# MIT-SPARK/Kimera-Semantics

Measured on NVIDIA H100. Metric: depth_frames_per_s, higher is better.
Workload: dtype f32

## Files before the change

### kimera_semantics_b200/csrc/ksg_api.cu

```cuda
#include <cuda_runtime.h>
#include <cub/cub.cuh>

#include <algorithm>
#include <climits>
#include <cmath>
#include <cstdio>
#include <cstdlib>
#include <cstring>
#include <memory>
#include <numeric>
#include <string>
#include <type_traits>
#include <unordered_map>
#include <unordered_set>
#include <utility>
#include <vector>

#include "../../include/ksg.h"
#include "ksg_kernels.cuh"
#include "ksg_chain.cuh"
#include "ksg_hot.cuh"
#include "ksg_bundle_order.cuh"
#include "ksg_fast.cuh"
#include "ksg_fast3.cuh"
// ... 136 lines not shown

}

struct ksg_integrator {
  ksg_config cfg{};
  DevCfg dc{};
  int device = 0;
  int sm_count = 132;
  cudaStream_t own_stream = nullptr;
  std::string err;
  int deferred_status = 0;

  MapRef map{};
  uint32_t ht_cap = 0;
  Luts h_luts{};
  Luts* d_luts = nullptr;
  Counters* d_cnt = nullptr;
  Counters* h_cnt = nullptr;
  int frame_stamp = 0;
  int64_t num_blocks = 0;
  int64_t last_blocks_touched = 0;

  int cap_points = 0;
  float4 *pt_pC = nullptr, *pt_pG = nullptr;
  uint8_t *pt_label = nullptr, *pt_flags = nullptr;
  uint32_t* pt_color = nullptr;
  uint64_t* pt_key = nullptr;
  uint8_t* flags8 = nullptr;
  int* pix_list = nullptr;
  int* point_of_seq = nullptr;
  uint32_t *sq_keys = nullptr, *sq_keys_out = nullptr;
  uint32_t *iota = nullptr;

  int *start_next = nullptr, *start_min = nullptr, *start_max = nullptr;
  uint32_t *start_table = nullptr;
  int *s_base = nullptr, *s_visits = nullptr;
  uint32_t *s_hmin = nullptr, *s_hmax = nullptr;
  uint8_t *clear_ff = nullptr, *clear_00 = nullptr;
  uint64_t set_offset = 0;
  int64_t reset_counter = 0;
  int* cast_seq = nullptr;
  float4* ray_param = nullptr;
  uint8_t *ray_label = nullptr, *ray_flags = nullptr;
  uint32_t* ray_color = nullptr;
  int* nsteps = nullptr;
  RayState* ray_state = nullptr;
  long long* ext_off = nullptr;
  Obs3 o3{};

  uint64_t* ks_sorted = nullptr;
  uint32_t* seq_sorted = nullptr;
  int *bstart = nullptr, *bundle_f = nullptr;
  float *hist = nullptr, *tmp = nullptr, *tmp4 = nullptr;
  uint64_t* b_key = nullptr;
  long long* b_base = nullptr;
  std::vector<std::pair<int, uint32_t>> bord_phases;
  uint32_t* bord_hash = nullptr;
  int* bundle_f2 = nullptr;
  int* bord_scratch = nullptr;
  unsigned long long* d_scan_tot = nullptr;
  BordBuf bord{};

  bool hot_enabled = false;
  HotSeg* d_hot_segs = nullptr;
  HotSeg* h_hot_segs = nullptr;
  int *d_hot_counts = nullptr;
  int *d_hot_chunk_seg = nullptr, *h_hot_chunk_seg = nullptr, *d_hot_guess = nullptr;
// ... 321 lines not shown
}
int finish_frame(ksg_integrator* h, ksg_frame_stats* stats) {
  while (h->n_pend > 1) { const int rc = finish_oldest(h, nullptr); if (rc) return rc; }
  if (h->n_pend == 1) return finish_oldest(h, stats);
  if (stats) fill_stats(h, stats);
  if (h->deferred_status) return h->fail(h->deferred_status, err_text(h->deferred_status));
  return KSG_OK;
}
int complete_frames(ksg_integrator* h) {
  KSG_CUDA(cudaSetDevice(h->device));
  KSG_CUDA(cudaDeviceSynchronize());
  return finish_frame(h, nullptr);
}

int advance_sets(ksg_integrator* h, cudaStream_t s) {
  if ((++h->reset_counter) >= h->cfg.clear_checks_every_n_frames) {
    h->reset_counter = 0;
    if (++h->set_offset >= 10000) {
      h->set_offset = 0;
      KSG_CUDA(cudaMemsetAsync(h->start_table, 0xFF, sizeof(uint32_t) * kSetSize, s));
      KSG_CUDA(cudaMemsetAsync(h->o3.table, 0xFF, sizeof(uint32_t) * kSetSize, s));
    }
  }
  return KSG_OK;
}

int integrate_fast(ksg_integrator* h, const InputDesc& in, const FrameIn& fin, const Xform& T, int cap, cudaStream_t s,
                   ksg_frame_stats* stats) {
  const bool sorted = h->cfg.integration_order_mode == KSG_ORDER_SORTED;
  { const int rcs = advance_sets(h, s); if (rcs) return rcs; }
  FastFrame f{};
  f.cfg = h->dc; f.T = T; f.in = fin; f.in.pix_list = nullptr; f.in.point_of_seq = nullptr;
  f.luts = h->d_luts; f.cnt = h->d_cnt; f.fc = h->d_fc; f.map = h->map;
  f.sb = StartBuf{h->start_next, h->start_min, h->start_max, h->start_table};
  f.set_offset = h->set_offset;
  f.capacity = cap;
  f.n_count_blocks = (cap + kCountBlock - 1) / kCountBlock;
  f.vec_ok = in.d_depth ? (((uintptr_t)in.d_depth % 16 == 0 && (uintptr_t)in.d_label_img % 4 == 0) ? 1 : 0) : 0;
  f.frame_stamp = h->frame_stamp;
  f.profile = (h->profiling && !h->profile_marks_only) ? 1 : 0;
  f.prof_marks = h->profiling ? 1 : 0;
  f.seq_of_i = sorted ? h->seq_of_i : nullptr;
  f.block_cnt = h->blk_cnt; f.block_off = h->blk_off; f.warp_cnt = h->warp_cnt; f.warp_off = h->warp_off;
  f.pt_pG = h->pt_pG; f.pt_label = h->pt_label; f.pt_flags = h->pt_flags; f.pt_color = h->pt_color; f.pt_key = h->pt_key;
  f.cast_flag = h->flags8;
  f.cast_seq = h->cast_seq; f.ray_param = h->ray_param; f.ray_label = h->ray_label; f.ray_flags = h->ray_flags; f.ray_color = h->ray_color;
  f.ray_state = h->ray_state; f.ext_off = h->ext_off;
  f.rec_cap = h->rec_cap; f.keys = h->keys32;
  f.tile_cnt = h->tile_cnt; f.tile_slot = h->tile_slot; f.tile_list = h->tile_list; f.tile_cap = h->tile_cap;
  f.o3 = h->o3;
  f.rayrec = h->rayrec; f.blk_run = h->blk_run;
  f.wl_listed = h->wl;
  f.wl_list[0] = h->wl + h->cap_points; f.wl_list[1] = h->wl + 2 * (size_t)h->cap_points;
  f.log_head = h->d_log_head; f.log_prior = h->d_log_prior; f.log_cap = h->log_cap;
  f.s_base = h->s_base; f.s_hmin = h->s_hmin; f.s_hmax = h->s_hmax; f.s_visits = h->s_visits;
  f.mixed_list = h->mixed_list; f.m_list = h->m_list;

  if (h->profiling) {
    cudaEventRecord(h->ev[0], s);
    KSG_CUDA(cudaMemsetAsync(h->d_fc->dbg, 0, sizeof(h->d_fc->dbg), s));
  }
  KSG_CUDA(cudaMemsetAsync(h->clear_ff, 0xFF, (size_t)kSetSize * 16, s));
  KSG_CUDA(cudaMemsetAsync(h->clear_00, 0x00, (size_t)kSetSize * 13, s));
  KSG_CUDA(cudaMemsetAsync(h->start_min, 0x7F, sizeof(int) * kSetSize, s));
  const int B = 256;
  ++h->n_launches;
  if (in.d_depth) k_fast_count<<<f.n_count_blocks, 256, 0, s>>>(f);
  else k_fast_reset<<<1, 1, 0, s>>>(f);
  if (sorted) {
    h->n_launches += 3;
    if (in.d_depth) k_fast_sqnorm<<<f.n_count_blocks, 256, 0, s>>>(f, h->sq_keys);
    else k_fast_sqnorm_points<<<grid_for(cap, B), B, 0, s>>>(f, h->sq_keys);
    k_fast_pad_keys<<<grid_for(cap, B), B, 0, s>>>(h->d_cnt, cap, h->sq_keys);
    size_t tb = h->cub_temp_bytes;
    ++h->n_libcalls;
    KSG_CUDA(cub::DeviceRadixSort::SortPairs(h->cub_temp, tb, h->sq_keys, h->sq_keys_out, h->iota, (uint32_t*)h->point_of_seq, cap, 0, 32, s));
    k_fast_invert_perm<<<grid_for(cap, B), B, 0, s>>>(h->d_cnt, (const uint32_t*)h->point_of_seq, h->seq_of_i);
  }
  ++h->n_launches;
  if (in.d_depth) k_fast_classify<true><<<f.n_count_blocks, 256, 0, s>>>(f);
  else k_fast_classify<false><<<grid_for(cap, B), B, 0, s>>>(f);
  ++h->n_launches;
  k_fast_start_eval3<<<(cap + kEvalBlock - 1) / kEvalBlock, kEvalBlock, 0, s>>>(f);
  if (h->profiling) cudaEventRecord(h->ev[1], s);
  {
    int max_sweeps = h->cap_points + 2;
    void* args[] = {(void*)&f, (void*)&max_sweeps};
    ++h->n_launches;
    KSG_CUDA(cudaLaunchCooperativeKernel((const void*)k_fast_solve3, dim3(h->solve_grid), dim3(h->solve_threads), args,
                                         (size_t)h->solve_smem, s));
  }
  if (h->profiling) cudaEventRecord(h->ev[2], s);
  {
    ApplySrc src{};
    src.param = h->ray_param; src.label = h->ray_label; src.color = h->ray_color; src.tmp = nullptr;
// ... 472 lines not shown
    h->h_luts.dynamic_label[l] = cfg->dynamic_label[l];
  }
  for (int i = 0; i < 1024; ++i) { h->h_luts.c2l_keys[i] = 0xFFFFFFFFu; h->h_luts.c2l_vals[i] = 0; }
  KSG_CUDA(res.device(&h->d_luts, 1));
  KSG_CUDA(cudaMemcpy(h->d_luts, &h->h_luts, sizeof(Luts), cudaMemcpyHostToDevice));

  h->ht_cap = 1024;
  while (h->ht_cap < 2u * (uint32_t)cfg->max_blocks) h->ht_cap <<= 1;
  if ((unsigned long long)h->ht_cap * dc.tiles_per_block >= (1ull << 32)) return h->fail(KSG_ERR_INVALID_ARGUMENT, "max_blocks too large");
  h->map.ht_mask = h->ht_cap - 1;
  h->map.max_blocks = cfg->max_blocks;
  h->map.new_cap = cfg->max_blocks;
  KSG_CUDA(res.device(&h->map.ht_keys, h->ht_cap));
  KSG_CUDA(res.device(&h->map.ht_slot, h->ht_cap));
  KSG_CUDA(res.device(&h->map.touched_stamp, h->ht_cap));
  KSG_CUDA(res.device(&h->map.touched_list, h->ht_cap));
  KSG_CUDA(res.device(&h->map.new_list, (size_t)cfg->max_blocks));
  KSG_CUDA(res.device(&h->map.slot_key, (size_t)cfg->max_blocks));
  KSG_CUDA(res.device(&h->map.pool, (size_t)dc.block_stride * (size_t)cfg->max_blocks));
  KSG_CUDA(res.device(&h->d_cnt, 1));
  KSG_CUDA(res.pinned(&h->h_cnt_base, 2));
  std::memset(h->h_cnt_base, 0, 2 * sizeof(Counters));
  h->h_cnt = h->h_cnt_base;
  for (int i = 0; i < 2; ++i) {
    KSG_CUDA(res.event(&h->ev_frame_s[i], cudaEventDisableTiming));
    KSG_CUDA(res.event(&h->ev_copy[i], cudaEventDisableTiming));
    KSG_CUDA(res.event(&h->ev_free[i], cudaEventDisableTiming));
  }
  KSG_CUDA(res.stream(&h->copy_stream));

  const size_t N = (size_t)cfg->max_points;
  h->cap_points = cfg->max_points;
  const bool fast = cfg->integrator_type == KSG_INTEGRATOR_FAST;
  KSG_CUDA(res.device(&h->pt_pC, N)); KSG_CUDA(res.device(&h->pt_pG, N));
  KSG_CUDA(res.device(&h->pt_label, N)); KSG_CUDA(res.device(&h->pt_flags, N));
  KSG_CUDA(res.device(&h->pt_color, N)); KSG_CUDA(res.device(&h->pt_key, N));
  KSG_CUDA(res.device(&h->flags8, 2 * N));
  KSG_CUDA(res.device(&h->pix_list, N));
  KSG_CUDA(res.device(&h->iota, N));
  k_iota<<<grid_for((long long)N, 256), 256>>>(h->iota, (int)N);
  if (cfg->integration_order_mode == KSG_ORDER_SORTED) {
    KSG_CUDA(res.device(&h->point_of_seq, N)); KSG_CUDA(res.device(&h->sq_keys, N)); KSG_CUDA(res.device(&h->sq_keys_out, N));
  }
  KSG_CUDA(res.device(&h->ray_param, N)); KSG_CUDA(res.device(&h->ray_flags, N)); KSG_CUDA(res.device(&h->nsteps, N));
  long long rec_cap = cfg->max_updates > 0 ? cfg->max_updates : (fast ? std::max<long long>(4ll << 20, 64ll * (long long)N) : (64ll << 20));
  if (fast) {
    KSG_CUDA(res.device(&h->start_next, N)); KSG_CUDA(res.device(&h->start_table, kSetSize));
    KSG_CUDA(res.device(&h->clear_ff, (size_t)kSetSize * 16));
    KSG_CUDA(res.device(&h->clear_00, (size_t)kSetSize * 13));
    h->s_base = (int*)h->clear_ff; h->start_max = h->s_base + kSetSize; h->s_hmin = (uint32_t*)(h->start_max + kSetSize);
    h->o3.head = (int*)(h->clear_ff + (size_t)kSetSize * 12);
    h->o3.slot_cnt = (int*)h->clear_00;
    h->s_hmax = (uint32_t*)(h->clear_00 + (size_t)kSetSize * 5); h->s_visits = (int*)(h->clear_00 + (size_t)kSetSize * 9);
    KSG_CUDA(res.device(&h->start_min, kSetSize));
    KSG_CUDA(res.device(&h->cast_seq, N));
    KSG_CUDA(res.device(&h->ray_label, N)); KSG_CUDA(res.device(&h->ray_color, N));
    KSG_CUDA(res.device(&h->ray_state, N)); KSG_CUDA(res.device(&h->ext_off, N * kExtSegs));
    long long ext = cfg->max_ray_steps > 0 ? cfg->max_ray_steps : std::max<long long>(16ll << 20, 64ll * (long long)N);
    Obs3& o3 = h->o3;
    o3.ext_base = (long long)N * kH0;
    o3.cand_cap = o3.ext_base + ext;
    if (o3.cand_cap >= 0x7FFFFFFFll) { o3.cand_cap = 0x7FFFFFFEll; }
    KSG_CUDA(res.device(&o3.cand, (size_t)o3.cand_cap));
    o3.ovf_cap = (int)std::min<long long>(std::max<long long>(1ll << 20, 4ll * (long long)N), 1ll << 28);
    KSG_CUDA(res.device(&o3.ovf, (size_t)o3.ovf_cap));
    KSG_CUDA(res.device(&o3.bkt, (size_t)kSetSize * kBkt3));
    KSG_CUDA(res.device(&o3.stamp_max, 2 * (size_t)kSetSize)); o3.stamp_min = o3.stamp_max + kSetSize;
    KSG_CUDA(res.device(&o3.table, kSetSize));
    KSG_CUDA(res.device(&h->rayrec, N));
    KSG_CUDA(res.device(&h->wl, 3 * N));
    KSG_CUDA(res.device(&h->mixed_list, N)); KSG_CUDA(res.device(&h->m_list, N));
    KSG_CUDA(res.device(&h->blk_run, (size_t)(o3.cand_cap / 16 + 16)));
  } else {
    KSG_CUDA(res.device(&h->ks_sorted, N)); KSG_CUDA(res.device(&h->seq_sorted, N));
    KSG_CUDA(res.device(&h->bstart, 2 * N)); KSG_CUDA(res.device(&h->bundle_f, N));
    KSG_CUDA(res.device(&h->hist, N * dc.C)); KSG_CUDA(res.device(&h->tmp, (N + 1) * dc.C));
    KSG_CUDA(res.device(&h->b_key, N)); KSG_CUDA(res.device(&h->b_base, N));
    KSG_CUDA(res.device(&h->d_scan_tot, 16));
    h->voxel_apply = cfg->apply_mode == 0 && !knobs.tile_apply;
    if (h->voxel_apply) {
      h->vq.long_cap = 4 * (rec_cap / kLongLen) + 64;
      h->vq.long_len = kLongLen;
      if (dc.C <= 32) {
        KSG_CUDA(res.device(&h->tmp4, (N + 1) * (size_t)((dc.C + 3) & ~3)));
// ... 1505 lines not shown
```

### kimera_semantics_b200/csrc/ksg_fast.cuh

```cuda
#pragma once
#include "ksg_kernels.cuh"

namespace ksg {

static constexpr int kCountBlock = 1024;
static constexpr int kEvalBlock = 512;
static constexpr int kSolveThreads = 1024;
static constexpr int kFastKeyCap = 4096;
static constexpr int kGroupThreads = 512;
static constexpr int kFastApplyThreads = 256;
static constexpr int kRecVoxMax = 1 << kRecVoxBits;
static constexpr int kTimelineSlots = 64;

struct FastCounters {
  unsigned int ticket_count, ticket_eval;
  unsigned int gridbar;
  int sweep_base;
  int sweeps_last;
  int tile_cursor;
  int n_tile_list;
  int pool_base;
  unsigned long long rec_cursor;
  int ovf_count;
  int n_mixed;
  int m_cursor;
  int log_count;
  int item_cursor;
  int wl_claim[4];
  int wl_count[4];
  long long timeline[kTimelineSlots];
  long long dbg[16];
};

struct TileDesc { uint32_t tk; int n; long long off; };
struct __align__(16) FastTile { long long off; int slot, tile, bx, by, bz, pad; };
struct __align__(16) FastItem { int tile, vox, lo, len; };

struct VoxelUpdate { int bx, by, bz; uint32_t lin_label; float dist, wgt; uint32_t rgba, srgba; };

struct StartBuf {
  int* next;
  int* smin;
  int* smax;
  const uint32_t* table;
};

struct Cand;
struct OvfEnt;
struct RayRec;
struct Obs3 {
  Cand* cand;
  long long ext_base, cand_cap;
  int* slot_cnt;
  uint64_t* bkt;
  int* head;
  OvfEnt* ovf;
  int ovf_cap;
  uint64_t* stamp_max;
  uint64_t* stamp_min;
  uint32_t* table;
};

struct FastFrame {
  DevCfg cfg;
  Xform T;
  FrameIn in;
  const Luts* luts;
  Counters* cnt;
  FastCounters* fc;
  MapRef map;
  StartBuf sb;
  uint64_t set_offset;
  int capacity;
  int n_count_blocks;
  int vec_ok;
  int frame_stamp;
  int profile;
  int prof_marks;
  const int* seq_of_i;
  int* block_cnt; int* block_off;
  int* warp_cnt; int* warp_off;
  float4* pt_pG; uint8_t* pt_label; uint8_t* pt_flags; uint32_t* pt_color; uint64_t* pt_key; uint8_t* cast_flag;
  int* cast_seq; float4* ray_param; uint8_t* ray_label; uint8_t* ray_flags; uint32_t* ray_color;
  RayState* ray_state; long long* ext_off;
  long long rec_cap;
  uint32_t* keys;
  int* tile_cnt;
  int* tile_slot;
  TileDesc* tile_list; long long tile_cap;
  Obs3 o3;
  RayRec* rayrec;
  int* blk_run;
  int* wl_listed;
  int* wl_list[2];
  VoxelUpdate* log_head; float* log_prior; int log_cap;
  int* s_visits;
  uint32_t *s_hmin, *s_hmax;
  int* s_base;
  int* mixed_list;
  int* m_list;
};

__device__ __forceinline__ int inv_mixed_index(int i, int n) {
  const int groups = n / 1024;
  if (groups * 1024 <= i) return i;
  return (i % 1024) * groups + i / 1024;
}

__device__ __forceinline__ int block_scan_array(const int* a, int* out, int n) {
  __shared__ int s_w[32];
  __shared__ int s_total;
  const int tid = threadIdx.x, lane = tid & 31, wid = tid >> 5;
  const int nthreads = blockDim.x, nwarps = nthreads >> 5;
  const int per = (((n + nthreads - 1) / nthreads) + 3) & ~3;
  const int i0 = min(n, tid * per), i1 = min(n, i0 + per);
// ... 32 lines not shown

__device__ __forceinline__ void load_depth4(const float* __restrict__ depth, int p0, int P, int vec_ok, float d[4], int& npx) {
  npx = P - p0; if (npx > 4) npx = 4; if (npx < 0) npx = 0;
  if (npx == 4 && vec_ok) { const float4 v = __ldg((const float4*)(depth + p0)); d[0] = v.x; d[1] = v.y; d[2] = v.z; d[3] = v.w; }
  else { for (int k = 0; k < 4; ++k) d[k] = (k < npx) ? __ldg(depth + p0 + k) : 0.0f; }
}

__global__ void __launch_bounds__(256) k_fast_count(FastFrame f) {
  __shared__ int s_w[8];
  __shared__ int s_last;
  const int tid = threadIdx.x, lane = tid & 31, wid = tid >> 5;
  const int p0 = blockIdx.x * kCountBlock + tid * 4;
  float d[4]; int npx;
  load_depth4(f.in.depth, p0, f.capacity, f.vec_ok, d, npx);
  int c = 0;
  for (int k = 0; k < 4; ++k) c += (k < npx && isfinite(d[k])) ? 1 : 0;
  for (int o = 16; o > 0; o >>= 1) c += __shfl_down_sync(0xffffffffu, c, o);
  if (lane == 0) s_w[wid] = c;
  __syncthreads();
  if (tid == 0) {
    int t = 0; for (int w = 0; w < 8; ++w) t += s_w[w];
    __stcg(&f.block_cnt[blockIdx.x], t);
    __threadfence();
    s_last = (atomicAdd(&f.fc->ticket_count, 1u) == (unsigned)(f.n_count_blocks - 1));
  }
  __syncthreads();
  if (!s_last) return;
  __threadfence();
  const int total = block_scan_array(f.block_cnt, f.block_off, f.n_count_blocks);
  if (tid == 0) { frame_counters_reset(f.cnt, total); f.fc->ticket_count = 0; }
}
__global__ void k_fast_reset(FastFrame f) { frame_counters_reset(f.cnt, f.capacity); }

__device__ __forceinline__ void fast_classify_one(const FastFrame& f, int seq, F3 pC, uint8_t label, uint32_t color, bool& valid) {
  const DevCfg& cfg = f.cfg;
  if ((int)label >= cfg.C) { set_err(f.cnt, 1 ); label = 0; }
  const float ray_distance = norm3(pC);
  valid = true;
  bool clearing = false;
  if (ray_distance < cfg.min_ray) valid = false;
  else if (ray_distance > cfg.max_ray) { if (cfg.allow_clear || f.in.freespace) clearing = true; else valid = false; }
  else clearing = f.in.freespace != 0;
  if (!(ray_distance == ray_distance)) valid = false;
  if (f.luts->dynamic_label[label]) valid = false;
  float w;
  if (cfg.const_weight) w = 1.0f;
  else { const float z = fabsf(pC.z); w = (z > kEps) ? 1.0f / (z * z) : 0.0f; }
  const F3 pG = xform_apply(f.T, pC);
  f.pt_pG[seq] = make_float4(pG.x, pG.y, pG.z, w);
  f.pt_label[seq] = label;
  f.pt_color[seq] = color;
  f.pt_flags[seq] = (valid ? 1 : 0) | (clearing ? 2 : 0);
  uint64_t key = ~0ull;
  if (valid) {
    const F3 sc = mul(pG, cfg.start_inv);
    if (!index_in_range(sc)) set_err(f.cnt, 5);
    const I3 g = grid_index(pG, cfg.start_inv);
    key = (uint64_t)index_hash(g) + f.set_offset;
    const uint32_t slot = (uint32_t)key & kSetMask, hi = (uint32_t)(key >> kSetBits);
    f.sb.next[seq] = atomicAdd(&f.s_visits[slot], 1);
    atomicMin(&f.sb.smin[slot], seq);
    atomicMax(&f.sb.smax[slot], seq);
    atomicMin(&f.s_hmin[slot], hi);
    atomicMax(&f.s_hmax[slot], hi);
  }
  f.pt_key[seq] = key;
}

template <bool DEPTH>
__global__ void __launch_bounds__(256) k_fast_classify(FastFrame f) {
  __shared__ int s_w[8];
  const int tid = threadIdx.x, lane = tid & 31, wid = tid >> 5;
  const int n = f.cnt->n_points;
  int nvalid = 0;
  if (DEPTH) {
    const int p0 = blockIdx.x * kCountBlock + tid * 4;
    float d[4]; int npx;
    load_depth4(f.in.depth, p0, f.capacity, f.vec_ok, d, npx);
    uint8_t lab[4] = {0, 0, 0, 0};
    if (npx == 4 && f.vec_ok) { const uchar4 v = __ldg((const uchar4*)(f.in.label_img + p0)); lab[0] = v.x; lab[1] = v.y; lab[2] = v.z; lab[3] = v.w; }
    else { for (int k = 0; k < npx; ++k) lab[k] = __ldg(f.in.label_img + p0 + k); }
    int c = 0;
    for (int k = 0; k < 4; ++k) c += (k < npx && isfinite(d[k])) ? 1 : 0;
    int incl = c;
    for (int o = 1; o < 32; o <<= 1) { const int v = __shfl_up_sync(0xffffffffu, incl, o); if (lane >= o) incl += v; }
    if (lane == 31) s_w[wid] = incl;
    __syncthreads();
    int base = f.block_off[blockIdx.x];
    for (int w = 0; w < wid; ++w) base += s_w[w];
    int i = base + incl - c;
    for (int k = 0; k < npx; ++k) {
      if (!isfinite(d[k])) continue;
      const int pix = p0 + k;
      const int v = pix / f.in.width, u = pix - v * f.in.width;
      const F3 pC = f3(((float)u - f.in.cx) * d[k] * f.in.constant_x, ((float)v - f.in.cy) * d[k] * f.in.constant_y, d[k] * f.in.z_scale);
      const int seq = f.seq_of_i ? f.seq_of_i[i] : inv_mixed_index(i, n);
      bool valid;
      fast_classify_one(f, seq, pC, lab[k], f.in.color_img ? f.in.color_img[pix] : f.luts->label_rgba[lab[k]], valid);
      nvalid += valid ? 1 : 0;
      ++i;
    }
  } else {
    const int i = blockIdx.x * blockDim.x + tid;
    if (i < n) {
      const FrameIn& in = f.in;
      const F3 pC = f3(in.xyz[3 * i], in.xyz[3 * i + 1], in.xyz[3 * i + 2]);
      uint32_t color = 0;
      uint8_t label = 0;
      if (in.rgba) color = (uint32_t)in.rgba[4 * i] | ((uint32_t)in.rgba[4 * i + 1] << 8) | ((uint32_t)in.rgba[4 * i + 2] << 16) | ((uint32_t)in.rgba[4 * i + 3] << 24);
      if (in.labels) label = in.labels[i];
      else if (in.rgba) {
        const uint32_t rgb = color & 0x00FFFFFFu;
        uint32_t hh = (rgb * 2654435761u) >> 22;
        for (int p = 0; p < 1024; ++p) {
          const uint32_t k = f.luts->c2l_keys[hh];
          if (k == rgb) { label = f.luts->c2l_vals[hh]; break; }
          if (k == 0xFFFFFFFFu) break;
          hh = (hh + 1) & 1023;
        }
      }
      if (!in.rgba) color = f.luts->label_rgba[label];
      const int seq = f.seq_of_i ? f.seq_of_i[i] : inv_mixed_index(i, n);
      bool valid;
      fast_classify_one(f, seq, pC, label, color, valid);
      nvalid = valid ? 1 : 0;
    }
  }
  for (int o = 16; o > 0; o >>= 1) nvalid += __shfl_down_sync(0xffffffffu, nvalid, o);
  if (lane == 0 && nvalid) atomicAdd(&f.cnt->n_valid, nvalid);
}

__global__ void __launch_bounds__(256) k_fast_sqnorm(FastFrame f, uint32_t* __restrict__ keys) {
  __shared__ int s_w[8];
  const int tid = threadIdx.x, lane = tid & 31, wid = tid >> 5;
  const int p0 = blockIdx.x * kCountBlock + tid * 4;
  float d[4]; int npx;
  load_depth4(f.in.depth, p0, f.capacity, f.vec_ok, d, npx);
  int c = 0;
  for (int k = 0; k < 4; ++k) c += (k < npx && isfinite(d[k])) ? 1 : 0;
  int incl = c;
  for (int o = 1; o < 32; o <<= 1) { const int v = __shfl_up_sync(0xffffffffu, incl, o); if (lane >= o) incl += v; }
  if (lane == 31) s_w[wid] = incl;
  __syncthreads();
  int base = f.block_off[blockIdx.x];
  for (int w = 0; w < wid; ++w) base += s_w[w];
  int i = base + incl - c;
  for (int k = 0; k < npx; ++k) {
    if (!isfinite(d[k])) continue;
    const int pix = p0 + k;
    const int v = pix / f.in.width, u = pix - v * f.in.width;
    const F3 pC = f3(((float)u - f.in.cx) * d[k] * f.in.constant_x, ((float)v - f.in.cy) * d[k] * f.in.constant_y, d[k] * f.in.z_scale);
    keys[i++] = __float_as_uint(dot3(pC, pC));
  }
}
__global__ void k_fast_sqnorm_points(FastFrame f, uint32_t* __restrict__ keys) {
  const int i = blockIdx.x * blockDim.x + threadIdx.x;
  if (i >= f.capacity) return;
  const F3 pC = f3(f.in.xyz[3 * i], f.in.xyz[3 * i + 1], f.in.xyz[3 * i + 2]);
  keys[i] = __float_as_uint(dot3(pC, pC));
}
__global__ void k_fast_pad_keys(const Counters* cnt, int capacity, uint32_t* __restrict__ keys) {
  const int i = blockIdx.x * blockDim.x + threadIdx.x;
  if (i < capacity && i >= cnt->n_points) keys[i] = 0xFFFFFFFFu;
}
__global__ void k_fast_invert_perm(const Counters* cnt, const uint32_t* __restrict__ point_of_seq, int* __restrict__ seq_of_i) {
  const int s = blockIdx.x * blockDim.x + threadIdx.x;
  if (s < cnt->n_points) seq_of_i[point_of_seq[s]] = s;
}

__global__ void __launch_bounds__(kEvalBlock) k_fast_start_eval3(FastFrame f) {
  const int seq = blockIdx.x * kEvalBlock + threadIdx.x;
  const int lane = threadIdx.x & 31;
  const StartBuf& sb = f.sb;
  uint8_t cast = 0;
  if (seq < f.cnt->n_points) {
    const uint64_t v = f.pt_key[seq];
    if (v != ~0ull) {
      const uint32_t slot = (uint32_t)v & kSetMask, hi = (uint32_t)(v >> kSetBits);
      if (sb.smin[slot] == seq) {
        cast = sb.table[slot] != hi;
        ((uint32_t*)sb.table)[slot] = (uint32_t)(f.pt_key[sb.smax[slot]] >> kSetBits);
        if (f.s_hmin[slot] != f.s_hmax[slot]) {
          f.s_base[slot] = atomicAdd(&f.fc->m_cursor, f.s_visits[slot]);
          f.mixed_list[atomicAdd(&f.fc->n_mixed, 1)] = (int)slot;
        }
      }
    }
  }
  if (seq < f.capacity) f.cast_flag[seq] = cast;
  const unsigned m = __ballot_sync(0xffffffffu, cast != 0);
  if (lane == 0) __stcg(&f.warp_cnt[seq >> 5], __popc(m));
  if (blockIdx.x == 0 && threadIdx.x == 0) f.fc->gridbar = 0;
}

__device__ __forceinline__ void warp_sort_i32(int* a, int n, int lane) {
  int n2 = 1;
  while (n2 < n) n2 <<= 1;
  const int half = n2 >> 1;
  for (int k = 2; k <= n2; k <<= 1) {
    const int hk = k >> 1;
    for (int t = lane; t < half; t += 32) {
      const int blk = t / hk, o = t - blk * hk;
      const int i = blk * k + o, p = blk * k + (k - 1 - o);
      if (p < n) { const int x = a[i], y = a[p]; if (x > y) { a[i] = y; a[p] = x; } }
    }
    __syncwarp();
    for (int j = k >> 2; j > 0; j >>= 1) {
      for (int t = lane; t < half; t += 32) {
        const int i = (t / j) * 2 * j + (t % j), p = i + j;
        if (p < n) { const int x = a[i], y = a[p]; if (x > y) { a[i] = y; a[p] = x; } }
      }
      __syncwarp();
    }
  }
// ... 262 lines not shown
```

### kimera_semantics_b200/csrc/ksg_fast3.cuh

```cuda
#pragma once
#include <cuda/atomic>
#include "ksg_fast.cuh"

namespace ksg {

struct __align__(16) Cand { uint64_t vkey; int pos; int tog; };
struct __align__(16) OvfEnt { uint64_t order_perf; uint32_t hi; int next; };
struct __align__(16) RayRec { int H, L, nsteps, eval_sweep; };
static constexpr int kBkt3 = 32;
static constexpr int kOvfPending = -2;
static constexpr int kSortPerWarp = 1024;

__device__ __forceinline__ Cand ld_cand(const Cand* p) {
  const int4 v = __ldcg((const int4*)p);
  Cand c; c.vkey = ((uint64_t)(uint32_t)v.y << 32) | (uint32_t)v.x; c.pos = v.z; c.tog = v.w;
  return c;
}
__device__ __forceinline__ void st_cand(Cand* p, uint64_t vkey, int pos, int tog) {
  __stcg((int4*)p, make_int4((int)(uint32_t)vkey, (int)(uint32_t)(vkey >> 32), pos, tog));
}
__device__ __forceinline__ void st_cand_state(Cand* p, int pos, int tog) { __stcg((int2*)p + 1, make_int2(pos, tog)); }
__device__ __forceinline__ uint64_t cand_value(uint64_t vkey, uint64_t offset) { return (uint64_t)index_hash(unpack_key(vkey)) + offset; }
__device__ __forceinline__ uint64_t make_entry(bool on, uint64_t order, uint64_t v) { return (on ? kEntPerf : 0ull) | (order << 13) | (v >> kSetBits); }
__device__ __forceinline__ long long cand_index3(const Obs3& o, const long long* ext_off, int r, int s) {
// ... 204 lines not shown
        cnt[k2] = lo;
      }
      const int rank = cnt[0] + cnt[1] + cnt[2];
      if (rank <= W) {
        I3 g; g.x = st.cx + sg0 * cnt[0]; g.y = st.cy + sg1 * cnt[1]; g.z = st.cz + sg2 * cnt[2];
        if (rank < W) { if (key_in_range(g)) sc->out[rank] = pack_key(g); else ok = false; }
        else { sc->endc[0] = cnt[0]; sc->endc[1] = cnt[1]; sc->endc[2] = cnt[2]; }
      }
    }
  }
  __syncwarp();
  const int e0 = sc->endc[0], e1 = sc->endc[1], e2 = sc->endc[2];
  st.cx += sg0 * e0; st.cy += sg1 * e1; st.cz += sg2 * e2;
  st.tn0 = sc->a[0][e0]; st.tn1 = sc->a[1][e1]; st.tn2 = sc->a[2][e2];
  return __all_sync(0xffffffffu, ok);
}

__device__ __forceinline__ void block_of_step(int s, int& s0, int& blen) {
  if (s < kH0) { s0 = 0; blen = kH0; return; }
  const int k = 31 - __clz(s >> 4);
  const int seg = kH0 << k;
  if (seg <= kWin) { s0 = seg; blen = seg; }
  else { s0 = seg + ((s - seg) & ~(kWin - 1)); blen = kWin; }
}

__device__ __forceinline__ void fast3_ray_setup(const FastFrame& f, int r, int n_cast) {
  const DevCfg& cfg = f.cfg;
  const Obs3& o = f.o3;
  int h = 0;
  const long long t_begin = f.profile ? clock64() : 0;
  long long t_ins = 0;
  if (r < n_cast) {
    const int seq = f.cast_seq[r];
    const float4 p = f.pt_pG[seq];
    const uint8_t fl = f.pt_flags[seq];
    f.ray_param[r] = p;
    f.ray_label[r] = f.pt_label[seq];
    f.ray_flags[r] = fl;
    f.ray_color[r] = f.pt_color[seq];
    if (f.profile) dbg_max(f, 12, clock64() - t_begin);
    Dda d;
    raycaster_init(d, f3(f.T.tx, f.T.ty, f.T.tz), f3(p.x, p.y, p.z), (fl & 2) != 0, cfg.carving != 0, cfg.max_ray, cfg.vsi, cfg.tp.trunc,
                   false);
    int n = d.length_in_steps + 1;
    if (!d.in_range || n >= (1 << kOrderStepBits)) { set_err(f.cnt, 5); n = 0; }
    if (f.profile) dbg_max(f, 13, clock64() - t_begin);
    h = n < kH0 ? n : kH0;
    const int l0 = h < cfg.maxc ? h : cfg.maxc;
    for (int s = 0; s < h; ++s) {
      const I3 g = dda_next(d);
      if (!key_in_range(g)) { set_err(f.cnt, 5); h = s; break; }
      const uint64_t vkey = pack_key(g);
      const long long ci = (long long)r * kH0 + s;
      int pos = -2;
      if (s < l0) {
        const long long t0 = f.profile ? clock64() : 0;
        const uint64_t v = (uint64_t)index_hash(g) + f.set_offset;
        pos = cand_insert3(f, (uint32_t)v & kSetMask, make_entry(true, ((uint64_t)r << kOrderStepBits) | (uint64_t)s, v));
        if (f.profile) t_ins += clock64() - t0;
      }
      st_cand(&o.cand[ci], vkey, pos, 0);
    }
    if (f.profile) dbg_max(f, 14, clock64() - t_begin);
    RayState st; save_state(st, d); f.ray_state[r] = st;
    RayRec rr; rr.H = h; rr.L = (h < l0) ? h : l0; rr.nsteps = (h < kH0 && h < n) ? h : n; rr.eval_sweep = 0;
    *(int4*)&f.rayrec[r] = make_int4(rr.H, rr.L, rr.nsteps, rr.eval_sweep);
  }
  warp_add(&f.cnt->ray_steps, (unsigned long long)h);
  if (f.profile) { dbg_max(f, 0, clock64() - t_begin); dbg_max(f, 1, t_ins); }
}

__device__ __forceinline__ int2 fast3_ray(const FastFrame& f, int r, int sweep, WarpDdaScratch* sc) {
// ... 215 lines not shown
      }
      if (htpos < 0) continue;
      const uint64_t rec = make_record(cfg, htpos, g, (uint32_t)r);
      const uint32_t tk = (uint32_t)(rec >> 32);
      if (PASS == 1) {
        if (atomicAdd(&f.tile_cnt[tk], 1) == 0) {
          const int idx = atomicAdd(&f.fc->n_tile_list, 1);
          if (idx < f.tile_cap) { f.tile_list[idx].tk = tk; f.tile_slot[tk] = idx; } else set_err(f.cnt, 4);
        }
      } else {
        const int at = atomicSub(&f.tile_cnt[tk], 1) - 1;
        const int idx = __ldcg(&f.tile_slot[tk]);
        if (idx >= 0 && idx < n_tiles && at >= 0) f.keys[__ldcg(&f.tile_list[idx].off) + at] = (uint32_t)rec;
      }
    }
  }
}

__global__ void __launch_bounds__(kSolveThreads, 1) k_fast_solve3(FastFrame f, int max_sweeps) {
  unsigned int epoch = 0;
  unsigned int* bar = &f.fc->gridbar;
  const int lane = threadIdx.x & 31;
  const int gtid0 = (((threadIdx.x >> 5) * gridDim.x + blockIdx.x) << 5) | lane;
  const int gthreads = gridDim.x * blockDim.x;
  Counters* cnt = f.cnt;
  const int n_points = cnt->n_points;
  int tl = 0;
  timeline_mark(f, tl++);
  extern __shared__ int s_sort[];
  const int n_mixed = ((volatile int*)&f.fc->n_mixed)[0];
  if (n_mixed > 0) {
    if (gtid0 == 0) f.fc->wl_claim[0] = 0;
    for (int seq = gtid0; seq < n_points; seq += gthreads) {
      const uint64_t v = f.pt_key[seq];
      if (v == ~0ull) continue;
      const uint32_t slot = (uint32_t)v & kSetMask;
      if (f.s_hmin[slot] != f.s_hmax[slot]) f.m_list[f.s_base[slot] + f.sb.next[seq]] = seq;
    }
    solve_barrier(bar, epoch);
    timeline_mark(f, 57);
    const int warps_total = gthreads >> 5;
    int* scratch = s_sort + (threadIdx.x >> 5) * kSortPerWarp;
    for (int mi = (threadIdx.x >> 5) * gridDim.x + blockIdx.x; mi < n_mixed;) {
      const int slot = f.mixed_list[mi];
      const int n = __ldcg(&f.s_visits[slot]);
      int* seg = f.m_list + __ldcg(&f.s_base[slot]);
      int* a = seg;
      if (n <= kSortPerWarp) { for (int i = lane; i < n; i += 32) scratch[i] = __ldcg(&seg[i]); a = scratch; }
      __syncwarp();
      warp_sort_i32(a, n, lane);
      for (int i = 1 + lane; i < n; i += 32) {
        const int pa = a[i - 1], pb = a[i];
        if (f.pt_key[pa] != f.pt_key[pb]) { f.cast_flag[pb] = 1; atomicAdd(&f.warp_cnt[pb >> 5], 1); }
      }
      __syncwarp();
      if (f.profile && lane == 0) { dbg_max(f, 8, n); dbg_add(f, 9, n); }
      int next = 0;
      if (lane == 0) next = warps_total + atomicAdd(&f.fc->wl_claim[0], 1);
      mi = __shfl_sync(0xffffffffu, next, 0);
    }
    solve_barrier(bar, epoch);
    timeline_mark(f, 58);
  }
  if (blockIdx.x == 0) {
    const int n_warps32 = (f.capacity + 31) >> 5;
    const int total = block_scan_array(f.warp_cnt, f.warp_off, n_warps32);
    if (threadIdx.x == 0) cnt->n_cast = total;
  }
  solve_barrier(bar, epoch);
  timeline_mark(f, 59);
  const int n_cast = ((volatile int*)&cnt->n_cast)[0];
  for (int base = (gtid0 & ~31); base < n_points; base += gthreads) {
    const int seq = base + lane;
    const bool c = seq < n_points && __ldcg(&f.cast_flag[seq]) != 0;
    const unsigned m = __ballot_sync(0xffffffffu, c);
    if (c) f.cast_seq[__ldcg(&f.warp_off[seq >> 5]) + __popc(m & ((1u << lane) - 1u))] = seq;
  }
  const int sweep_base0 = ((volatile int*)&f.fc->sweep_base)[0];
  if (gtid0 == 0) for (int k = 0; k < 4; ++k) { f.fc->wl_claim[k] = 0; f.fc->wl_count[k] = 0; }
  solve_barrier(bar, epoch);
  timeline_mark(f, tl++);
  for (int r0 = (gtid0 & ~31); r0 < n_cast; r0 += gthreads) fast3_ray_setup(f, r0 + lane, n_cast);
  solve_barrier(bar, epoch);
  timeline_mark(f, tl++);
  int sweep = (sweep_base0 + 4) & ~3;
  bool converged = n_cast == 0;
  int it = 0;
  while (!converged && it < max_sweeps) {
    ++it;
    ++sweep;
    fast3_sweep(f, sweep, it, (WarpDdaScratch*)(s_sort + (threadIdx.x >> 5) * kSortPerWarp));
    solve_barrier(bar, epoch);
    if (tl < kTimelineSlots - 12) timeline_mark(f, tl++);
    const int changed = ((volatile int*)cnt->changed)[sweep & 3];
    const int err = ((volatile int*)&cnt->err)[0];
    if (err) break;
    converged = !changed;
  }
  const bool failed = !converged;
  const int gtid = solve_gtid_fresh();
  if (gtid == 0) {
    cnt->last_sweep = sweep;
    f.fc->sweep_base = sweep;
    f.fc->sweeps_last = it;
    if (failed && !((volatile int*)&cnt->err)[0]) set_err(cnt, 2 );
    if (f.prof_marks) f.fc->timeline[kTimelineSlots - 1] = tl;
  }
  tl = kTimelineSlots - 12;
  timeline_mark(f, tl++);
  if (!failed) fast3_walk_performed<1>(f, ((volatile int*)&cnt->n_cast)[0], 0, gtid);
  solve_barrier(bar, epoch);
  timeline_mark(f, tl++);
  timeline_mark(f, tl++);
  const bool ok = ((volatile int*)&cnt->err)[0] == 0 && !failed;
  const int n_new_all = ((volatile int*)&cnt->n_new_blocks)[0];
  const int n_new = n_new_all < f.map.new_cap ? n_new_all : f.map.new_cap;
  const int pool_base = ((volatile int*)&cnt->pool_count)[0];
  const int n_tiles = (int)min((long long)((volatile int*)&f.fc->n_tile_list)[0], f.tile_cap);
  for (int base = (gtid & ~31); base < n_tiles; base += gthreads) {
    const int idx = base + lane;
    int n = 0;
    uint32_t tk = 0;
    if (idx < n_tiles) { tk = f.tile_list[idx].tk; n = __ldcg(&f.tile_cnt[tk]); }
    const long long off = (long long)warp_alloc(&f.fc->rec_cursor, (unsigned long long)n);
    if (idx < n_tiles) {
      const int pos = (int)(tk / (uint32_t)f.cfg.tiles_per_block);
      const int old = atomicExch(&f.map.touched_stamp[pos], f.frame_stamp);
      if (old != f.frame_stamp) f.map.touched_list[atomicAdd(&cnt->n_blocks_touched, 1)] = pos;
      const bool owned = f.cfg.shard_count <= 1 ||
                         tile_owner(f.map.ht_keys[pos], (int)(tk % (uint32_t)f.cfg.tiles_per_block), f.cfg.shard_count) == f.cfg.shard_rank;
      if (off + n > f.rec_cap) { set_err(cnt, 4); n = 0; }
      f.tile_list[idx].n = owned ? n : -n;
      f.tile_list[idx].off = off;
    }
  }
  if (ok) fast_block_init(f, n_new, pool_base);
  solve_barrier(bar, epoch);
  timeline_mark(f, tl++);
  const bool ok2 = ((volatile int*)&cnt->err)[0] == 0 && !failed;
// ... 21 lines not shown
```

Baseline: 2146.

## Pack per-point data into AoS struct and warp-aggregate start-set atomics

```diff
diff --git a/kimera_semantics_b200/csrc/ksg_api.cu b/kimera_semantics_b200/csrc/ksg_api.cu
--- a/kimera_semantics_b200/csrc/ksg_api.cu
+++ b/kimera_semantics_b200/csrc/ksg_api.cu
@@ -192,7 +192,8 @@
   uint32_t *sq_keys = nullptr, *sq_keys_out = nullptr;
   uint32_t *iota = nullptr;
 
-  int *start_next = nullptr, *start_min = nullptr, *start_max = nullptr;
+  FastPoint* fast_pts = nullptr;
+  int *start_min = nullptr, *start_max = nullptr;
   uint32_t *start_table = nullptr;
   int *s_base = nullptr, *s_visits = nullptr;
   uint32_t *s_hmin = nullptr, *s_hmax = nullptr;
@@ -580,7 +581,7 @@
   FastFrame f{};
   f.cfg = h->dc; f.T = T; f.in = fin; f.in.pix_list = nullptr; f.in.point_of_seq = nullptr;
   f.luts = h->d_luts; f.cnt = h->d_cnt; f.fc = h->d_fc; f.map = h->map;
-  f.sb = StartBuf{h->start_next, h->start_min, h->start_max, h->start_table};
+  f.sb = StartBuf{h->start_min, h->start_max, h->start_table};
   f.set_offset = h->set_offset;
   f.capacity = cap;
   f.n_count_blocks = (cap + kCountBlock - 1) / kCountBlock;
@@ -590,7 +591,7 @@
   f.prof_marks = h->profiling ? 1 : 0;
   f.seq_of_i = sorted ? h->seq_of_i : nullptr;
   f.block_cnt = h->blk_cnt; f.block_off = h->blk_off; f.warp_cnt = h->warp_cnt; f.warp_off = h->warp_off;
-  f.pt_pG = h->pt_pG; f.pt_label = h->pt_label; f.pt_flags = h->pt_flags; f.pt_color = h->pt_color; f.pt_key = h->pt_key;
+  f.pts = h->fast_pts;
   f.cast_flag = h->flags8;
   f.cast_seq = h->cast_seq; f.ray_param = h->ray_param; f.ray_label = h->ray_label; f.ray_flags = h->ray_flags; f.ray_color = h->ray_color;
   f.ray_state = h->ray_state; f.ext_off = h->ext_off;
@@ -608,7 +609,7 @@
     cudaEventRecord(h->ev[0], s);
     KSG_CUDA(cudaMemsetAsync(h->d_fc->dbg, 0, sizeof(h->d_fc->dbg), s));
   }
-  KSG_CUDA(cudaMemsetAsync(h->clear_ff, 0xFF, (size_t)kSetSize * 16, s));
+  KSG_CUDA(cudaMemsetAsync(h->clear_ff, 0xFF, (size_t)kSetSize * 12, s));
   KSG_CUDA(cudaMemsetAsync(h->clear_00, 0x00, (size_t)kSetSize * 13, s));
   KSG_CUDA(cudaMemsetAsync(h->start_min, 0x7F, sizeof(int) * kSetSize, s));
   const int B = 256;
@@ -1147,9 +1148,11 @@
   const size_t N = (size_t)cfg->max_points;
   h->cap_points = cfg->max_points;
   const bool fast = cfg->integrator_type == KSG_INTEGRATOR_FAST;
-  KSG_CUDA(res.device(&h->pt_pC, N)); KSG_CUDA(res.device(&h->pt_pG, N));
-  KSG_CUDA(res.device(&h->pt_label, N)); KSG_CUDA(res.device(&h->pt_flags, N));
-  KSG_CUDA(res.device(&h->pt_color, N)); KSG_CUDA(res.device(&h->pt_key, N));
+  if (!fast) {
+    KSG_CUDA(res.device(&h->pt_pC, N)); KSG_CUDA(res.device(&h->pt_pG, N));
+    KSG_CUDA(res.device(&h->pt_label, N)); KSG_CUDA(res.device(&h->pt_flags, N));
+    KSG_CUDA(res.device(&h->pt_color, N)); KSG_CUDA(res.device(&h->pt_key, N));
+  }
   KSG_CUDA(res.device(&h->flags8, 2 * N));
   KSG_CUDA(res.device(&h->pix_list, N));
   KSG_CUDA(res.device(&h->iota, N));
@@ -1160,11 +1163,12 @@
   KSG_CUDA(res.device(&h->ray_param, N)); KSG_CUDA(res.device(&h->ray_flags, N)); KSG_CUDA(res.device(&h->nsteps, N));
   long long rec_cap = cfg->max_updates > 0 ? cfg->max_updates : (fast ? std::max<long long>(4ll << 20, 64ll * (long long)N) : (64ll << 20));
   if (fast) {
-    KSG_CUDA(res.device(&h->start_next, N)); KSG_CUDA(res.device(&h->start_table, kSetSize));
-    KSG_CUDA(res.device(&h->clear_ff, (size_t)kSetSize * 16));
+    KSG_CUDA(res.device(&h->fast_pts, N)); KSG_CUDA(res.device(&h->start_table, kSetSize));
+    KSG_CUDA(res.device(&h->clear_ff, (size_t)kSetSize * 12));
     KSG_CUDA(res.device(&h->clear_00, (size_t)kSetSize * 13));
-    h->s_base = (int*)h->clear_ff; h->start_max = h->s_base + kSetSize; h->s_hmin = (uint32_t*)(h->start_max + kSetSize);
-    h->o3.head = (int*)(h->clear_ff + (size_t)kSetSize * 12);
+    KSG_CUDA(res.device(&h->s_base, kSetSize));
+    h->start_max = (int*)h->clear_ff; h->s_hmin = (uint32_t*)(h->start_max + kSetSize);
+    h->o3.head = (int*)(h->clear_ff + (size_t)kSetSize * 8);
     h->o3.slot_cnt = (int*)h->clear_00;
     h->s_hmax = (uint32_t*)(h->clear_00 + (size_t)kSetSize * 5); h->s_visits = (int*)(h->clear_00 + (size_t)kSetSize * 9);
     KSG_CUDA(res.device(&h->start_min, kSetSize));
diff --git a/kimera_semantics_b200/csrc/ksg_fast.cuh b/kimera_semantics_b200/csrc/ksg_fast.cuh
--- a/kimera_semantics_b200/csrc/ksg_fast.cuh
+++ b/kimera_semantics_b200/csrc/ksg_fast.cuh
@@ -38,8 +38,14 @@
 
 struct VoxelUpdate { int bx, by, bz; uint32_t lin_label; float dist, wgt; uint32_t rgba, srgba; };
 
+struct __align__(32) FastPoint {
+  float4 pG;
+  uint64_t key;
+  uint32_t color;
+  uint8_t label, flags, pad[2];
+};
+
 struct StartBuf {
-  int* next;
   int* smin;
   int* smax;
   const uint32_t* table;
@@ -80,7 +86,7 @@
   const int* seq_of_i;
   int* block_cnt; int* block_off;
   int* warp_cnt; int* warp_off;
-  float4* pt_pG; uint8_t* pt_label; uint8_t* pt_flags; uint32_t* pt_color; uint64_t* pt_key; uint8_t* cast_flag;
+  FastPoint* pts; uint8_t* cast_flag;
   int* cast_seq; float4* ray_param; uint8_t* ray_label; uint8_t* ray_flags; uint32_t* ray_color;
   RayState* ray_state; long long* ext_off;
   long long rec_cap;
@@ -179,11 +185,17 @@
 }
 __global__ void k_fast_reset(FastFrame f) { frame_counters_reset(f.cnt, f.capacity); }
 
-__device__ __forceinline__ void fast_classify_one(const FastFrame& f, int seq, F3 pC, uint8_t label, uint32_t color, bool& valid) {
+__device__ __forceinline__ void st_point(FastPoint* p, F3 pG, float w, uint64_t key, uint32_t color, uint8_t label, uint8_t flags) {
+  int4* q = (int4*)p;
+  q[0] = make_int4(__float_as_int(pG.x), __float_as_int(pG.y), __float_as_int(pG.z), __float_as_int(w));
+  q[1] = make_int4((int)(uint32_t)key, (int)(uint32_t)(key >> 32), (int)color, (int)((uint32_t)label | ((uint32_t)flags << 8)));
+}
+
+__device__ __forceinline__ uint64_t fast_classify_one(const FastFrame& f, int seq, F3 pC, uint8_t label, uint32_t color) {
   const DevCfg& cfg = f.cfg;
   if ((int)label >= cfg.C) { set_err(f.cnt, 1 ); label = 0; }
   const float ray_distance = norm3(pC);
-  valid = true;
+  bool valid = true;
   bool clearing = false;
   if (ray_distance < cfg.min_ray) valid = false;
   else if (ray_distance > cfg.max_ray) { if (cfg.allow_clear || f.in.freespace) clearing = true; else valid = false; }
@@ -194,24 +206,32 @@
   if (cfg.const_weight) w = 1.0f;
   else { const float z = fabsf(pC.z); w = (z > kEps) ? 1.0f / (z * z) : 0.0f; }
   const F3 pG = xform_apply(f.T, pC);
-  f.pt_pG[seq] = make_float4(pG.x, pG.y, pG.z, w);
-  f.pt_label[seq] = label;
-  f.pt_color[seq] = color;
-  f.pt_flags[seq] = (valid ? 1 : 0) | (clearing ? 2 : 0);
   uint64_t key = ~0ull;
   if (valid) {
     const F3 sc = mul(pG, cfg.start_inv);
     if (!index_in_range(sc)) set_err(f.cnt, 5);
     const I3 g = grid_index(pG, cfg.start_inv);
     key = (uint64_t)index_hash(g) + f.set_offset;
-    const uint32_t slot = (uint32_t)key & kSetMask, hi = (uint32_t)(key >> kSetBits);
-    f.sb.next[seq] = atomicAdd(&f.s_visits[slot], 1);
-    atomicMin(&f.sb.smin[slot], seq);
-    atomicMax(&f.sb.smax[slot], seq);
-    atomicMin(&f.s_hmin[slot], hi);
-    atomicMax(&f.s_hmax[slot], hi);
-  }
-  f.pt_key[seq] = key;
+  }
+  st_point(&f.pts[seq], pG, w, key, color, label, (uint8_t)((valid ? 1 : 0) | (clearing ? 2 : 0)));
+  return key;
+}
+
+__device__ __forceinline__ void start_visits_warp(const FastFrame& f, uint64_t key, int seq) {
+  const bool valid = key != ~0ull;
+  const unsigned vm = __ballot_sync(0xffffffffu, valid);
+  if (!valid) return;
+  const uint32_t slot = (uint32_t)key & kSetMask, hi = (uint32_t)(key >> kSetBits);
+  const unsigned grp = __match_any_sync(vm, slot);
+  const int smin = __reduce_min_sync(grp, seq), smax = __reduce_max_sync(grp, seq);
+  const uint32_t hmin = __reduce_min_sync(grp, hi), hmax = __reduce_max_sync(grp, hi);
+  if ((int)(threadIdx.x & 31) == __ffs(grp) - 1) {
+    atomicAdd(&f.s_visits[slot], __popc(grp));
+    atomicMin(&f.sb.smin[slot], smin);
+    atomicMax(&f.sb.smax[slot], smax);
+    atomicMin(&f.s_hmin[slot], hmin);
+    atomicMax(&f.s_hmax[slot], hmax);
+  }
 }
 
 template <bool DEPTH>
@@ -221,34 +241,45 @@
   const int n = f.cnt->n_points;
   int nvalid = 0;
   if (DEPTH) {
-    const int p0 = blockIdx.x * kCountBlock + tid * 4;
-    float d[4]; int npx;
-    load_depth4(f.in.depth, p0, f.capacity, f.vec_ok, d, npx);
-    uint8_t lab[4] = {0, 0, 0, 0};
-    if (npx == 4 && f.vec_ok) { const uchar4 v = __ldg((const uchar4*)(f.in.label_img + p0)); lab[0] = v.x; lab[1] = v.y; lab[2] = v.z; lab[3] = v.w; }
-    else { for (int k = 0; k < npx; ++k) lab[k] = __ldg(f.in.label_img + p0 + k); }
+    const int p0 = blockIdx.x * kCountBlock + wid * 128 + lane;
+    float d[4];
+    uint8_t lab[4];
+    unsigned fin[4];
     int c = 0;
-    for (int k = 0; k < 4; ++k) c += (k < npx && isfinite(d[k])) ? 1 : 0;
-    int incl = c;
-    for (int o = 1; o < 32; o <<= 1) { const int v = __shfl_up_sync(0xffffffffu, incl, o); if (lane >= o) incl += v; }
-    if (lane == 31) s_w[wid] = incl;
+#pragma unroll
+    for (int k = 0; k < 4; ++k) {
+      const int pix = p0 + 32 * k;
+      const bool in = pix < f.capacity;
+      d[k] = in ? __ldg(f.in.depth + pix) : 0.0f;
+      lab[k] = in ? __ldg(f.in.label_img + pix) : 0;
+      fin[k] = __ballot_sync(0xffffffffu, in && isfinite(d[k]));
+      c += __popc(fin[k]);
+    }
+    if (lane == 0) s_w[wid] = c;
     __syncthreads();
-    int base = f.block_off[blockIdx.x];
-    for (int w = 0; w < wid; ++w) base += s_w[w];
-    int i = base + incl - c;
-    for (int k = 0; k < npx; ++k) {
-      if (!isfinite(d[k])) continue;
-      const int pix = p0 + k;
-      const int v = pix / f.in.width, u = pix - v * f.in.width;
-      const F3 pC = f3(((float)u - f.in.cx) * d[k] * f.in.constant_x, ((float)v - f.in.cy) * d[k] * f.in.constant_y, d[k] * f.in.z_scale);
-      const int seq = f.seq_of_i ? f.seq_of_i[i] : inv_mixed_index(i, n);
-      bool valid;
-      fast_classify_one(f, seq, pC, lab[k], f.in.color_img ? f.in.color_img[pix] : f.luts->label_rgba[lab[k]], valid);
-      nvalid += valid ? 1 : 0;
-      ++i;
+    int i = f.block_off[blockIdx.x];
+    for (int w = 0; w < wid; ++w) i += s_w[w];
+    const unsigned below = (1u << lane) - 1u;
+#pragma unroll
+    for (int k = 0; k < 4; ++k) {
+      uint64_t key = ~0ull;
+      int seq = 0;
+      if ((fin[k] >> lane) & 1u) {
+        const int pix = p0 + 32 * k;
+        const int v = pix / f.in.width, u = pix - v * f.in.width;
+        const F3 pC = f3(((float)u - f.in.cx) * d[k] * f.in.constant_x, ((float)v - f.in.cy) * d[k] * f.in.constant_y, d[k] * f.in.z_scale);
+        const int ik = i + __popc(fin[k] & below);
+        seq = f.seq_of_i ? f.seq_of_i[ik] : inv_mixed_index(ik, n);
+        key = fast_classify_one(f, seq, pC, lab[k], f.in.color_img ? f.in.color_img[pix] : f.luts->label_rgba[lab[k]]);
+        nvalid += key != ~0ull ? 1 : 0;
+      }
+      start_visits_warp(f, key, seq);
+      i += __popc(fin[k]);
     }
   } else {
     const int i = blockIdx.x * blockDim.x + tid;
+    uint64_t key = ~0ull;
+    int seq = 0;
     if (i < n) {
       const FrameIn& in = f.in;
       const F3 pC = f3(in.xyz[3 * i], in.xyz[3 * i + 1], in.xyz[3 * i + 2]);
@@ -267,11 +298,11 @@
         }
       }
       if (!in.rgba) color = f.luts->label_rgba[label];
-      const int seq = f.seq_of_i ? f.seq_of_i[i] : inv_mixed_index(i, n);
-      bool valid;
-      fast_classify_one(f, seq, pC, label, color, valid);
-      nvalid = valid ? 1 : 0;
-    }
+      seq = f.seq_of_i ? f.seq_of_i[i] : inv_mixed_index(i, n);
+      key = fast_classify_one(f, seq, pC, label, color);
+      nvalid = key != ~0ull ? 1 : 0;
+    }
+    start_visits_warp(f, key, seq);
   }
   for (int o = 16; o > 0; o >>= 1) nvalid += __shfl_down_sync(0xffffffffu, nvalid, o);
   if (lane == 0 && nvalid) atomicAdd(&f.cnt->n_valid, nvalid);
@@ -321,12 +352,12 @@
   const StartBuf& sb = f.sb;
   uint8_t cast = 0;
   if (seq < f.cnt->n_points) {
-    const uint64_t v = f.pt_key[seq];
+    const uint64_t v = f.pts[seq].key;
     if (v != ~0ull) {
       const uint32_t slot = (uint32_t)v & kSetMask, hi = (uint32_t)(v >> kSetBits);
       if (sb.smin[slot] == seq) {
         cast = sb.table[slot] != hi;
-        ((uint32_t*)sb.table)[slot] = (uint32_t)(f.pt_key[sb.smax[slot]] >> kSetBits);
+        ((uint32_t*)sb.table)[slot] = (uint32_t)(f.pts[sb.smax[slot]].key >> kSetBits);
         if (f.s_hmin[slot] != f.s_hmax[slot]) {
           f.s_base[slot] = atomicAdd(&f.fc->m_cursor, f.s_visits[slot]);
           f.mixed_list[atomicAdd(&f.fc->n_mixed, 1)] = (int)slot;
diff --git a/kimera_semantics_b200/csrc/ksg_fast3.cuh b/kimera_semantics_b200/csrc/ksg_fast3.cuh
--- a/kimera_semantics_b200/csrc/ksg_fast3.cuh
+++ b/kimera_semantics_b200/csrc/ksg_fast3.cuh
@@ -260,12 +260,13 @@
   long long t_ins = 0;
   if (r < n_cast) {
     const int seq = f.cast_seq[r];
-    const float4 p = f.pt_pG[seq];
-    const uint8_t fl = f.pt_flags[seq];
+    const int4 q = ((const int4*)&f.pts[seq])[1];
+    const float4 p = f.pts[seq].pG;
+    const uint8_t fl = (uint8_t)((uint32_t)q.w >> 8);
     f.ray_param[r] = p;
-    f.ray_label[r] = f.pt_label[seq];
+    f.ray_label[r] = (uint8_t)q.w;
     f.ray_flags[r] = fl;
-    f.ray_color[r] = f.pt_color[seq];
+    f.ray_color[r] = (uint32_t)q.z;
     if (f.profile) dbg_max(f, 12, clock64() - t_begin);
     Dda d;
     raycaster_init(d, f3(f.T.tx, f.T.ty, f.T.tz), f3(p.x, p.y, p.z), (fl & 2) != 0, cfg.carving != 0, cfg.max_ray, cfg.vsi, cfg.tp.trunc,
@@ -547,10 +548,10 @@
   if (n_mixed > 0) {
     if (gtid0 == 0) f.fc->wl_claim[0] = 0;
     for (int seq = gtid0; seq < n_points; seq += gthreads) {
-      const uint64_t v = f.pt_key[seq];
+      const uint64_t v = f.pts[seq].key;
       if (v == ~0ull) continue;
       const uint32_t slot = (uint32_t)v & kSetMask;
-      if (f.s_hmin[slot] != f.s_hmax[slot]) f.m_list[f.s_base[slot] + f.sb.next[seq]] = seq;
+      if (f.s_hmin[slot] != f.s_hmax[slot]) f.m_list[atomicAdd(&f.s_base[slot], 1)] = seq;
     }
     solve_barrier(bar, epoch);
     timeline_mark(f, 57);
@@ -559,14 +560,14 @@
     for (int mi = (threadIdx.x >> 5) * gridDim.x + blockIdx.x; mi < n_mixed;) {
       const int slot = f.mixed_list[mi];
       const int n = __ldcg(&f.s_visits[slot]);
-      int* seg = f.m_list + __ldcg(&f.s_base[slot]);
+      int* seg = f.m_list + (__ldcg(&f.s_base[slot]) - n);
       int* a = seg;
       if (n <= kSortPerWarp) { for (int i = lane; i < n; i += 32) scratch[i] = __ldcg(&seg[i]); a = scratch; }
       __syncwarp();
       warp_sort_i32(a, n, lane);
       for (int i = 1 + lane; i < n; i += 32) {
         const int pa = a[i - 1], pb = a[i];
-        if (f.pt_key[pa] != f.pt_key[pb]) { f.cast_flag[pb] = 1; atomicAdd(&f.warp_cnt[pb >> 5], 1); }
+        if (f.pts[pa].key != f.pts[pb].key) { f.cast_flag[pb] = 1; atomicAdd(&f.warp_cnt[pb >> 5], 1); }
       }
       __syncwarp();
       if (f.profile && lane == 0) { dbg_max(f, 8, n); dbg_add(f, 9, n); }
@@ -606,7 +607,7 @@
     ++sweep;
     fast3_sweep(f, sweep, it, (WarpDdaScratch*)(s_sort + (threadIdx.x >> 5) * kSortPerWarp));
     solve_barrier(bar, epoch);
-    if (tl < kTimelineSlots - 12) timeline_mark(f, tl++);
+    if (tl + it <= kTimelineSlots - 12) timeline_mark(f, tl + it - 1);
     const int changed = ((volatile int*)cnt->changed)[sweep & 3];
     const int err = ((volatile int*)&cnt->err)[0];
     if (err) break;
@@ -619,7 +620,7 @@
     f.fc->sweep_base = sweep;
     f.fc->sweeps_last = it;
     if (failed && !((volatile int*)&cnt->err)[0]) set_err(cnt, 2 );
-    if (f.prof_marks) f.fc->timeline[kTimelineSlots - 1] = tl;
+    if (f.prof_marks) f.fc->timeline[kTimelineSlots - 1] = min(tl + it, kTimelineSlots - 12);
   }
   tl = kTimelineSlots - 12;
   timeline_mark(f, tl++);
```

Result: faster. 2281, median of 6 (+6.3%).
